# suoych/KEDs

Measured on AMD Instinct MI355X. Metric: query-images/sec (encode+0.5M top-10) ViT-L/14, higher is better.
Workload: dtype bf16/fp16 operands, fp32 accumulate; 1 GPU; ViT-L/14 encode_image (224x224 synthetic, random-init weights) + exact top-10 over a synthetic unit-norm 0.5M x 768 database; batch_per_gpu=128, global_batch=128, db_rows=500000, dim=768, k=10, parallelism=dp1 encoders + 1-way row-sharded scan

## Files before the change

### keds_amd/csrc/elementwise.hip

```cpp
#include "keds_common.h"
#include <math.h>

namespace {

constexpr float LN_EPS = 1e-5f;
constexpr int LN_MAXV = 8;

template <int OUT, int NV>
__global__ __launch_bounds__(256) void layernorm_kernel(const float* __restrict__ x, long long x_stride,
                                                        const int* __restrict__ row_map, int row_mul,
                                                        const float* __restrict__ gamma,
                                                        const float* __restrict__ beta, void* __restrict__ out,
                                                        int rows, int dim, long long pair_plane) {
    const int r = blockIdx.x * 4 + (threadIdx.x >> 6);
    const int lane = threadIdx.x & 63;
    if (r >= rows) return;
    const int rm = row_map ? row_map[r] : 0;
    const bool bad_row = row_map && (unsigned)rm >= (unsigned)row_mul;
    const long long src = (long long)r * row_mul + (bad_row ? 0 : rm);
    const float* p = x + src * x_stride;
    constexpr int MAXV = NV > 0 ? NV : LN_MAXV;
    f32x4 v[MAXV], gg[MAXV], bb[MAXV];
#pragma unroll
    for (int j = 0; j < MAXV; ++j) {
// ... 221 lines not shown
    float acc0 = 0.f, acc1 = 0.f, acc2 = 0.f;
    for (int y = ylo; y < yhi; ++y) {
        const float wy = pil_bicubic((y - yc + 0.5f) * yss) / wys;
        float h0 = 0.f, h1 = 0.f, h2 = 0.f;
        if (RW == W) {
            const unsigned char* p = src + ((size_t)y * W + (ox + left)) * 3;
            h0 = p[0]; h1 = p[1]; h2 = p[2];
        } else {
            const unsigned char* row = src + (size_t)y * W * 3;
            for (int x = xlo; x < xhi; ++x) {
                const float wx = pil_bicubic((x - xc + 0.5f) * xss) / wxs;
                h0 += wx * row[x * 3];
                h1 += wx * row[x * 3 + 1];
                h2 += wx * row[x * 3 + 2];
            }
            h0 = clip8(h0); h1 = clip8(h1); h2 = clip8(h2);
        }
        if (RH == H) {
            if (y == oy + top) { acc0 = h0; acc1 = h1; acc2 = h2; }
        } else {
            acc0 += wy * h0; acc1 += wy * h1; acc2 += wy * h2;
        }
    }
    if (RH != H) { acc0 = clip8(acc0); acc1 = clip8(acc1); acc2 = clip8(acc2); }
    const size_t plane = (size_t)n_px * n_px;
    float* o = out + (size_t)b * 3 * plane + (size_t)oy * n_px + ox;
    o[0] = (acc0 * (1.f / 255.f) - m0) / s0;
    o[plane] = (acc1 * (1.f / 255.f) - m1) / s1;
    o[2 * plane] = (acc2 * (1.f / 255.f) - m2) / s2;
}

__global__ __launch_bounds__(256) void preprocess_pil_kernel(const unsigned char* __restrict__ img, int B, int H, int W,
                                                             int n_px, int need_h, int need_v, int left, int top,
                                                             const int* __restrict__ xb, const int* __restrict__ xk, int ksx,
                                                             const int* __restrict__ yb, const int* __restrict__ yk, int ksy,
                                                             float m0, float m1, float m2, float s0, float s1, float s2,
                                                             float* __restrict__ out, unsigned char* __restrict__ out_u8) {
    const int idx = blockIdx.x * 256 + threadIdx.x;
    if (idx >= B * n_px * n_px) return;
    const int b = idx / (n_px * n_px), rem = idx - b * n_px * n_px;
    const int oy = rem / n_px, ox = rem - oy * n_px;
    const unsigned char* src = img + (size_t)b * H * W * 3;
    const int x0 = need_h ? xb[2 * ox] : ox + left, xn = need_h ? xb[2 * ox + 1] : 1;
    const int y0 = need_v ? yb[2 * oy] : oy + top, yn = need_v ? yb[2 * oy + 1] : 1;
    const int* kx = xk + (size_t)ox * ksx;
    const int* ky = yk + (size_t)oy * ksy;
    auto clip8 = [](int v) { v >>= 22; return v < 0 ? 0 : (v > 255 ? 255 : v); };
    int a0 = 1 << 21, a1 = 1 << 21, a2 = 1 << 21;
    int r0 = 0, r1 = 0, r2 = 0;
    for (int y = 0; y < yn; ++y) {
        const unsigned char* row = src + ((size_t)(y0 + y) * W + x0) * 3;
        int h0, h1, h2;
        if (need_h) {
            h0 = h1 = h2 = 1 << 21;
            for (int x = 0; x < xn; ++x) {
                const int k = kx[x];
                h0 += k * row[3 * x];
                h1 += k * row[3 * x + 1];
                h2 += k * row[3 * x + 2];
            }
            h0 = clip8(h0); h1 = clip8(h1); h2 = clip8(h2);
        } else {
            h0 = row[0]; h1 = row[1]; h2 = row[2];
        }
        if (need_v) {
            const int k = ky[y];
            a0 += k * h0; a1 += k * h1; a2 += k * h2;
        } else {
            r0 = h0; r1 = h1; r2 = h2;
        }
    }
    if (need_v) { r0 = clip8(a0); r1 = clip8(a1); r2 = clip8(a2); }
    const size_t plane = (size_t)n_px * n_px;
    float* o = out + (size_t)b * 3 * plane + (size_t)oy * n_px + ox;
    o[0] = ((float)r0 / 255.0f - m0) / s0;
    o[plane] = ((float)r1 / 255.0f - m1) / s1;
    o[2 * plane] = ((float)r2 / 255.0f - m2) / s2;
    if (out_u8) {
        unsigned char* u = out_u8 + ((size_t)b * plane + (size_t)oy * n_px + ox) * 3;
        u[0] = (unsigned char)r0; u[1] = (unsigned char)r1; u[2] = (unsigned char)r2;
    }
}

template <typename T>
__global__ __launch_bounds__(256) void im2col_kernel(const float* __restrict__ img, T* __restrict__ out, int R,
                                                     int P, int Kpad) {
    const int g = R / P;
    const int row = blockIdx.x;
    const int b = row / (g * g), pi = row % (g * g);
    const int py = pi / g, px = pi % g;
    const int kreal = 3 * P * P;
    const float* base = img + (size_t)b * 3 * R * R;
    for (int k = threadIdx.x; k < Kpad; k += 256) {
        float v = 0.f;
        if (k < kreal) {
            const int ch = k / (P * P), rem = k % (P * P);
            const int ky = rem / P, kx = rem % P;
            v = base[(size_t)ch * R * R + (size_t)(py * P + ky) * R + px * P + kx];
        }
        out[(size_t)row * Kpad + k] = (T)v;
    }
}

__global__ void cls_rows_kernel(float* __restrict__ x, const float* __restrict__ cls, const float* __restrict__ pos,
                                int B, int S, int d) {
    const int i = blockIdx.x * blockDim.x + threadIdx.x;
    if (i >= B * d) return;
    const int b = i / d, j = i % d;
    x[(size_t)b * S * d + j] = cls[j] + pos[j];
}

__global__ __launch_bounds__(256) void embed_tokens_kernel(const int* __restrict__ tokens,
                                                           const float* __restrict__ table,
                                                           const float* __restrict__ pos,
                                                           const float* __restrict__ img_tokens, int n_tok,
                                                           int insert_col, float* __restrict__ x, int L, int Lx, int d,
                                                           const int* __restrict__ seq_off) {
    const int b = blockIdx.x / Lx, t = blockIdx.x % Lx;
    size_t orow = (size_t)b * Lx + t;
    if (seq_off) {
        const int r0 = seq_off[b];
        if (t >= seq_off[b + 1] - r0) return;
        orow = (size_t)r0 + t;
    }
    const float* src;
    if (img_tokens && t >= insert_col && t < insert_col + n_tok) {
        src = img_tokens + ((size_t)b * n_tok + (t - insert_col)) * d;
    } else {
        const int col = (img_tokens && t >= insert_col + n_tok) ? t - (n_tok - 1) : t;
        src = table + (size_t)tokens[(size_t)b * L + col] * d;
    }
    const float* pe = pos + (size_t)t * d;
    float* o = x + orow * d;
    for (int i = threadIdx.x * 4; i < d; i += 1024)
        *reinterpret_cast<f32x4*>(o + i) =
            *reinterpret_cast<const f32x4*>(src + i) + *reinterpret_cast<const f32x4*>(pe + i);
}

__global__ __launch_bounds__(256) void l2norm_kernel(const float* __restrict__ x, float* __restrict__ out, int rows,
                                                     int dim) {
    const int r = blockIdx.x * 4 + (threadIdx.x >> 6);
    const int lane = threadIdx.x & 63;
    if (r >= rows) return;
    const float* p = x + (size_t)r * dim;
    float s = 0.f;
    for (int i = lane; i < dim; i += 64) s += p[i] * p[i];
    const float nrm = sqrtf(wave_sum(s));
    for (int i = lane; i < dim; i += 64) out[(size_t)r * dim + i] = p[i] / nrm;
}

__global__ __launch_bounds__(256) void mix_kernel(const float* __restrict__ a, const float* __restrict__ b, float wa,
                                                  float wb, float* __restrict__ an, float* __restrict__ bn,
                                                  float* __restrict__ mix, int rows, int dim) {
    const int r = blockIdx.x * 4 + (threadIdx.x >> 6);
    const int lane = threadIdx.x & 63;
    if (r >= rows) return;
    const float* pa = a + (size_t)r * dim;
    const float* pb = b + (size_t)r * dim;
    float sa = 0.f, sb = 0.f;
    for (int i = lane; i < dim; i += 64) {
        sa += pa[i] * pa[i];
        sb += pb[i] * pb[i];
    }
    const float na = sqrtf(wave_sum(sa)), nb = sqrtf(wave_sum(sb));
    float sm = 0.f;
    for (int i = lane; i < dim; i += 64) {
        const float m = wa * (pa[i] / na) + wb * (pb[i] / nb);
        sm += m * m;
    }
    const float nm = sqrtf(wave_sum(sm));
    for (int i = lane; i < dim; i += 64) {
        const float va = pa[i] / na, vb = pb[i] / nb;
        an[(size_t)r * dim + i] = va;
        bn[(size_t)r * dim + i] = vb;
        mix[(size_t)r * dim + i] = (wa * va + wb * vb) / nm;
    }
}

template <typename T>
__global__ void cast16_kernel(const float* __restrict__ x, T* __restrict__ out, long long n) {
    typedef __attribute__((ext_vector_type(4))) T t4;
    long long i = (blockIdx.x * (long long)blockDim.x + threadIdx.x) * 4;
    const long long step = (long long)gridDim.x * blockDim.x * 4;
// ... 170 lines not shown
    KedsProfScope prof(KEDS_PROF_OTHER, (hipStream_t)stream);
    const long long threads = (long long)rows * (cols / 8);
    split_f16_pair_kernel<<<(unsigned)((threads + 255) / 256), 256, 0, (hipStream_t)stream>>>(x, ld, rows, cols, (f16_t*)out, plane, overflow, 1.0f);
    return keds_check_launch("split_f16_pair_kernel");
}

extern "C" int keds_split_f16_weight(const float* w, int64_t n, int k, void* out, int64_t plane, int* w_exp, void* stream) {
    KEDS_REQUIRE(w && out && w_exp && n > 0 && k > 0 && k % 8 == 0 && plane >= n * k, "keds_split_f16_weight: bad argument");
    hipStream_t st = (hipStream_t)stream;
    unsigned* dmax = nullptr;
    if (hipMalloc(&dmax, sizeof(unsigned)) != hipSuccess) {
        keds_set_error("keds_split_f16_weight: out of device memory");
        return KEDS_E_LAUNCH;
    }
    unsigned hmax = 0;
    int rc = KEDS_OK;
    if (hipMemsetAsync(dmax, 0, sizeof(unsigned), st) != hipSuccess) rc = KEDS_E_LAUNCH;
    if (!rc) {
        absmax_bits_kernel<<<1024, 256, 0, st>>>(w, (long long)n * k, dmax);
        rc = keds_check_launch("absmax_bits_kernel");
    }
    if (!rc && (hipMemcpyAsync(&hmax, dmax, sizeof(unsigned), hipMemcpyDeviceToHost, st) != hipSuccess ||
                hipStreamSynchronize(st) != hipSuccess))
        rc = KEDS_E_LAUNCH;
    (void)hipFree(dmax);
    if (rc) {
        if (rc == KEDS_E_LAUNCH) keds_set_error("keds_split_f16_weight: device error while reading max |W|");
        return rc;
    }
    KEDS_REQUIRE(hmax < 0x7F800000u, "keds_split_f16_weight: the weight matrix holds a non-finite value");
    int e = 0;
    if (hmax) {
        const int lg = (int)(hmax >> 23) - 127;
        e = 13 - lg;
        if (e > 40) e = 40;
        if (e < -100) e = -100;
    }
    *w_exp = e;
    const long long threads = (long long)n * (k / 8);
    split_f16_pair_kernel<<<(unsigned)((threads + 255) / 256), 256, 0, st>>>(w, k, n, k, (f16_t*)out, plane, nullptr, ldexpf(1.0f, e));
    return keds_check_launch("split_f16_pair_kernel");
}

extern "C" int keds_layernorm(const float* x, int64_t x_stride, const float* gamma, const float* beta, void* out,
                              int out_f32, int rows, int dim, void* stream) {
    KEDS_REQUIRE(x && gamma && beta && out && rows > 0, "keds_layernorm: bad argument");
    KEDS_REQUIRE(ln_dim_ok(dim), "keds_layernorm: dim %d unsupported", dim);
    KEDS_REQUIRE(x_stride % 4 == 0, "keds_layernorm: row stride must be a multiple of 4");
    return keds_layernorm_impl(x, x_stride, nullptr, 1, gamma, beta, out, out_f32 ? 1 : 0, rows, dim, (hipStream_t)stream);
}

extern "C" int keds_layernorm_ex(const float* x, int64_t x_stride, const float* gamma, const float* beta, void* out,
                                 int out_type, int rows, int dim, void* stream) {
    KEDS_REQUIRE(out_type >= 0 && out_type <= 2, "keds_layernorm_ex: out_type %d (0 bf16, 1 fp32, 2 fp16)", out_type);
    KEDS_REQUIRE(x && gamma && beta && out && rows > 0, "keds_layernorm: bad argument");
    KEDS_REQUIRE(ln_dim_ok(dim), "keds_layernorm: dim %d unsupported", dim);
    KEDS_REQUIRE(x_stride % 4 == 0, "keds_layernorm: row stride must be a multiple of 4");
    return keds_layernorm_impl(x, x_stride, nullptr, 1, gamma, beta, out, out_type, rows, dim, (hipStream_t)stream);
}

extern "C" int keds_layernorm_rows(const float* x, int64_t x_stride, const int32_t* row_map, int row_mul, const float* gamma,
                                   const float* beta, void* out, int out_type, int rows, int dim, void* stream) {
    KEDS_REQUIRE(out_type >= 0 && out_type <= 2, "keds_layernorm_rows: out_type %d (0 bf16, 1 fp32, 2 fp16)", out_type);
    KEDS_REQUIRE(x && gamma && beta && out && rows > 0 && row_mul > 0, "keds_layernorm_rows: bad argument");
    KEDS_REQUIRE(ln_dim_ok(dim), "keds_layernorm_rows: dim %d unsupported", dim);
    KEDS_REQUIRE(x_stride % 4 == 0, "keds_layernorm_rows: row stride must be a multiple of 4");
    return keds_layernorm_impl(x, x_stride, row_map, row_mul, gamma, beta, out, out_type, rows, dim, (hipStream_t)stream);
}

extern "C" int keds_layernorm_pair(const float* x, int64_t x_stride, const float* gamma, const float* beta, void* out, int64_t plane,
                                   int rows, int dim, int form, void* stream) {
    KEDS_REQUIRE(x && gamma && beta && out && rows > 0 && (form == 0 || form == 1), "keds_layernorm_pair: bad argument");
    KEDS_REQUIRE(ln_dim_ok(dim), "keds_layernorm_pair: dim %d unsupported", dim);
    KEDS_REQUIRE(x_stride % 4 == 0, "keds_layernorm_pair: row stride must be a multiple of 4");
    KEDS_REQUIRE(plane % 4 == 0 && plane >= (int64_t)rows * dim, "keds_layernorm_pair: plane must be a multiple of 4 and hold rows * dim");
    return keds_layernorm_pair_impl(x, x_stride, gamma, beta, out, plane, rows, dim, (hipStream_t)stream, form);
}

extern "C" int keds_layernorm_pair_last_form(void) { return tl_ln_pair_form; }

extern "C" int keds_im2col_ex(const float* image, void* out, int out_f16, int B, int R, int P, int Kpad, void* stream) {
    KEDS_REQUIRE(image && out && B > 0 && P > 0 && R % P == 0, "keds_im2col: bad argument");
    KEDS_REQUIRE(Kpad >= 3 * P * P && Kpad % 64 == 0, "keds_im2col: Kpad must cover 3*P*P and be a multiple of 64");
    const int g = R / P;
    KedsProfScope prof(KEDS_PROF_OTHER, (hipStream_t)stream);
    if (out_f16) im2col_kernel<f16_t><<<B * g * g, 256, 0, (hipStream_t)stream>>>(image, (f16_t*)out, R, P, Kpad);
    else im2col_kernel<bf16_t><<<B * g * g, 256, 0, (hipStream_t)stream>>>(image, (bf16_t*)out, R, P, Kpad);
    return keds_check_launch("im2col_kernel");
}

extern "C" int keds_im2col(const float* image, void* out, int B, int R, int P, int Kpad, void* stream) {
    return keds_im2col_ex(image, out, 0, B, R, P, Kpad, stream);
}

int keds_cls_rows_impl(float* x, const float* cls, const float* pos, int B, int S, int d, hipStream_t st) {
    cls_rows_kernel<<<(B * d + 255) / 256, 256, 0, st>>>(x, cls, pos, B, S, d);
    return keds_check_launch("cls_rows_kernel");
}


extern "C" int keds_cls_rows(float* x, const float* cls, const float* pos, int B, int S, int d, void* stream) {
    KEDS_REQUIRE(x && cls && pos && B > 0 && S > 0 && d > 0, "keds_cls_rows: bad argument");
    return keds_cls_rows_impl(x, cls, pos, B, S, d, (hipStream_t)stream);
}

extern "C" int keds_embed_tokens_ex(const int32_t* tokens, const float* table, const float* pos, const float* img_tokens, int n_tok,
                                    int insert_col, float* x, int B, int L, int Lx, int d, const int32_t* seq_off, void* stream) {
    return keds_embed_tokens_impl(tokens, table, pos, img_tokens, n_tok, insert_col, x, B, L, Lx, d, stream, seq_off);
}

extern "C" int keds_embed_tokens(const int32_t* tokens, const float* table, const float* pos, const float* img_tokens,
                                 int n_tok, int insert_col, float* x, int B, int L, int d, void* stream) {
    return keds_embed_tokens_impl(tokens, table, pos, img_tokens, n_tok, insert_col, x, B, L, L, d, stream);
}

int keds_embed_tokens_impl(const int32_t* tokens, const float* table, const float* pos, const float* img_tokens,
                           int n_tok, int insert_col, float* x, int B, int L, int Lx, int d, void* stream, const int32_t* seq_off) {
    KEDS_REQUIRE(tokens && table && pos && x && B > 0 && L > 0 && Lx > 0 && Lx <= L, "keds_embed_tokens: bad argument");
    KEDS_REQUIRE(d % 4 == 0, "keds_embed_tokens: d must be a multiple of 4");
    if (img_tokens) {
        KEDS_REQUIRE(n_tok >= 1 && insert_col >= 0 && insert_col + n_tok <= L,
                     "keds_embed_tokens: splice [%d,%d) outside the context of %d", insert_col, insert_col + n_tok, L);
    }
    KedsProfScope prof(KEDS_PROF_OTHER, (hipStream_t)stream);
    embed_tokens_kernel<<<B * Lx, 256, 0, (hipStream_t)stream>>>(tokens, table, pos, img_tokens, n_tok, insert_col, x, L,
                                                                  Lx, d, seq_off);
    return keds_check_launch("embed_tokens_kernel");
}

extern "C" size_t keds_readout_workspace_bytes(int B, int d) {
    return keds_align_up((size_t)B, 128) * d * 2;
}

extern "C" int keds_readout(const float* x, int S, const int32_t* row, const float* gamma, const float* beta,
                            const void* proj_t, float* out, int B, int d, int E, int normalize, void* workspace,
                            size_t workspace_bytes, void* stream) {
    KEDS_REQUIRE(x && gamma && beta && proj_t && out && workspace && B > 0, "keds_readout: bad argument");
    KEDS_REQUIRE(ln_dim_ok(d), "keds_readout: d %d unsupported", d);
    if (workspace_bytes < keds_readout_workspace_bytes(B, d)) {
        keds_set_error("keds_readout: workspace too small");
        return KEDS_E_WORKSPACE;
    }
    return keds_run_readout(x, S, row, gamma, beta, proj_t, out, B, d, E, normalize, workspace, (hipStream_t)stream);
}

extern "C" int keds_l2_normalize(const float* x, float* out, int rows, int dim, void* stream) {
    KEDS_REQUIRE(x && out && rows > 0 && dim > 0, "keds_l2_normalize: bad argument");
    l2norm_kernel<<<(rows + 3) / 4, 256, 0, (hipStream_t)stream>>>(x, out, rows, dim);
    return keds_check_launch("l2norm_kernel");
}

extern "C" int keds_mix_normalize(const float* a, const float* b, float wa, float wb, float* a_n, float* b_n,
                                  float* mix, int rows, int dim, void* stream) {
    KEDS_REQUIRE(a && b && a_n && b_n && mix && rows > 0 && dim > 0, "keds_mix_normalize: bad argument");
    mix_kernel<<<(rows + 3) / 4, 256, 0, (hipStream_t)stream>>>(a, b, wa, wb, a_n, b_n, mix, rows, dim);
    return keds_check_launch("mix_kernel");
}

extern "C" int keds_cast_bf16(const float* x, void* out, int64_t count, void* stream) {
    KEDS_REQUIRE(x && out && count > 0, "keds_cast_bf16: bad argument");
    long long blocks = (count / 4 + 255) / 256;
    if (blocks > 4096) blocks = 4096;
    if (blocks < 1) blocks = 1;
    cast16_kernel<bf16_t><<<(unsigned)blocks, 256, 0, (hipStream_t)stream>>>(x, (bf16_t*)out, count);
    return keds_check_launch("cast16_kernel<bf16>");
}

extern "C" int keds_cast_f16(const float* x, void* out, int64_t count, void* stream) {
    KEDS_REQUIRE(x && out && count > 0, "keds_cast_f16: bad argument");
    long long blocks = (count / 4 + 255) / 256;
// ... 148 lines not shown
```

### keds_amd/csrc/gemm.hip

```cpp
#include "keds_common.h"
#include <math.h>
#include "gemm_shared.h"
#include "gemm_quad_gen.h"

#ifndef KEDS_QUAD_AUX_X
#define KEDS_QUAD_AUX_X 0
#endif
#ifndef KEDS_QUAD_AUX_W
#define KEDS_QUAD_AUX_W 0
#endif

namespace {

constexpr int BM = 128, BN = 128, BK = 64;
constexpr int TILE_BYTES = 128 * BK * 2;
constexpr int BUF_BYTES = 2 * TILE_BYTES;


__device__ __forceinline__ float qgelu(float x) {
    return x * __builtin_amdgcn_rcpf(1.0f + __builtin_amdgcn_exp2f(-2.4554669595930157f * x));
}

template <int EPI>
__device__ __forceinline__ void epilogue_store(f32x4 v0, f32x4 v1, void* __restrict__ out, int m, int n, int N,
// ... 268 lines not shown
            if constexpr (ND > 0) {
                if (16 * H + p * 8 + mi >= 32 - ND && defer) {
                    pend[16 * H + p * 8 + mi - (32 - ND)] = ov;
                    continue;
                }
            }
            keds_store16<KEDS_ST_LN>(ov, tile_out, off);
        }
    }
    if constexpr (epi_out_f16(EPI)) f16_range_flag(guard, rmax);
}
template <int ND>
__device__ __forceinline__ void quad_flush_pending(const u32x4* __restrict__ pend, char* __restrict__ tile_out, int N, int wm, int wn2,
                                                   int g, int c, int i0, int i1) {
    int r0 = 128 * wm + c;
    asm volatile("" : "+v"(r0));
#pragma unroll
    for (int i = 0; i < ND; ++i) {
        if (i < i0 || i >= i1) continue;
        const int s_ = 32 - ND + i, h = s_ >> 4, p = (s_ >> 3) & 1, mi = s_ & 7;
        const unsigned off = ((unsigned)(r0 + 16 * mi) * (unsigned)N + (unsigned)(64 * (2 * wn2 + h) + 32 * p + 8 * g)) * 2u;
        keds_store16<KEDS_ST_LN>(pend[i], tile_out, off);
    }
}

template <bool REDUCE = true>
__device__ __forceinline__ void pair_resid_epilogue(f32x4 (&acc)[4][8], const char* __restrict__ side, void* __restrict__ out,
                                                    int m0, int n0, int N, int wm, int wn, int g, int c,
                                                    keds_stat_t* __restrict__ stats, char* __restrict__ red) {
    const int r0 = 128 * wm + c;
    char* tile = reinterpret_cast<char*>(out) + ((size_t)m0 * N + n0) * 2;
    const int nl = 64 * wn + 8 * g;
    f16x8 r[2][8];
#if KEDS_LD_RESID_AUX
    const auto trs = __builtin_amdgcn_make_buffer_rsrc(tile, 0, 0x7FFFFFFF, 0x00020000);
#endif
#pragma unroll
    for (int p = 0; p < 2; ++p)
#pragma unroll
        for (int mi = 0; mi < 8; ++mi) {
#if KEDS_LD_RESID_AUX
            r[p][mi] = __builtin_bit_cast(f16x8, __builtin_amdgcn_raw_buffer_load_b128(
                           trs, (int)(((unsigned)(r0 + 16 * mi) * (unsigned)N + (unsigned)(nl + 32 * p)) * 2u), 0, KEDS_LD_RESID_AUX));
#else
            r[p][mi] = *reinterpret_cast<const f16x8*>(tile + ((unsigned)(r0 + 16 * mi) * (unsigned)N + (unsigned)(nl + 32 * p)) * 2u);
#endif
        }
    f32x4 b[2][2];
#pragma unroll
    for (int p = 0; p < 2; ++p) {
        b[p][0] = *reinterpret_cast<const f32x4*>(side + 2048 + (nl + 32 * p) * 4);
        b[p][1] = *reinterpret_cast<const f32x4*>(side + 2048 + (nl + 32 * p) * 4 + 16);
    }
    f32x2* rw = reinterpret_cast<f32x2*>(red) + wn * 256 + r0;
#pragma unroll
    for (int mi = 0; mi < 8; ++mi) {
        f32x4 sv = f32x4{0.f, 0.f, 0.f, 0.f}, qv = sv;
#pragma unroll
        for (int p = 0; p < 2; ++p) {
            const f16x8 q = r[p][mi];
            const f32x4 v0 = f32x4{(float)q[0], (float)q[1], (float)q[2], (float)q[3]} + (acc[2 * p][mi] + b[p][0]);
            const f32x4 v1 = f32x4{(float)q[4], (float)q[5], (float)q[6], (float)q[7]} + (acc[2 * p + 1][mi] + b[p][1]);
            const f16x8 ov = f16x8{(f16_t)v0[0], (f16_t)v0[1], (f16_t)v0[2], (f16_t)v0[3], (f16_t)v1[0], (f16_t)v1[1], (f16_t)v1[2], (f16_t)v1[3]};
            keds_store16<KEDS_ST_RESID>(ov, tile, ((unsigned)(r0 + 16 * mi) * (unsigned)N + (unsigned)(nl + 32 * p)) * 2u);
            sv = sv + (v0 + v1);
            qv = qv + (v0 * v0 + v1 * v1);
        }
        float s = (sv[0] + sv[1]) + (sv[2] + sv[3]), ss = (qv[0] + qv[1]) + (qv[2] + qv[3]);
        s = rows_sum(s);
        ss = rows_sum(ss);
        if (stats && g == 0) rw[16 * mi] = f32x2{s, ss};
    }
    if constexpr (REDUCE) {
        if (stats) {
            __syncthreads();
            const int t = threadIdx.x;
            if (t < 256) {
                const f32x2* rr = reinterpret_cast<const f32x2*>(red) + t;
                const f32x2 a = rr[0], b = rr[256], c2 = rr[512], d = rr[768];
                keds_stat_add(stats + 2 * (size_t)(m0 + t), (a[0] + b[0]) + (c2[0] + d[0]), (a[1] + b[1]) + (c2[1] + d[1]));
            }
        }
    }
}

__device__ __forceinline__ void pair_resid_epilogue_acc(f32x4 (&acc)[4][8], void* __restrict__ out, int m0, int n0, int N,
                                                        int wm, int wn, int g, int c, keds_stat_t* __restrict__ stats,
                                                        char* __restrict__ red) {
    const int r0 = 128 * wm + c;
    char* tile = reinterpret_cast<char*>(out) + ((size_t)m0 * N + n0) * 2;
    const int nl = 64 * wn + 8 * g;
    f32x2* rw = reinterpret_cast<f32x2*>(red) + wn * 256 + r0;
#pragma unroll
    for (int mi = 0; mi < 8; ++mi) {
        float s = 0.f, ss = 0.f;
#pragma unroll
        for (int p = 0; p < 2; ++p) {
            const f32x4 v0 = acc[2 * p][mi], v1 = acc[2 * p + 1][mi];
            const f16x8 ov = f16x8{(f16_t)v0[0], (f16_t)v0[1], (f16_t)v0[2], (f16_t)v0[3], (f16_t)v1[0], (f16_t)v1[1], (f16_t)v1[2], (f16_t)v1[3]};
            *reinterpret_cast<f16x8*>(tile + ((unsigned)(r0 + 16 * mi) * (unsigned)N + (unsigned)(nl + 32 * p)) * 2u) = ov;
            s += sum8(v0, v1);
            ss += sum8(v0 * v0, v1 * v1);
        }
        s = rows_sum(s);
        ss = rows_sum(ss);
        if (stats && g == 0) rw[16 * mi] = f32x2{s, ss};
    }
    if (stats) {
        __syncthreads();
        const int t = threadIdx.x;
        if (t < 256) {
            const f32x2* rr = reinterpret_cast<const f32x2*>(red) + t;
            const f32x2 a = rr[0], b = rr[256], c2 = rr[512], d = rr[768];
            keds_stat_add(stats + 2 * (size_t)(m0 + t), (a[0] + b[0]) + (c2[0] + d[0]), (a[1] + b[1]) + (c2[1] + d[1]));
        }
    }
}

template <int N>
__device__ __forceinline__ void small_wait_barrier() {
    asm volatile("s_waitcnt vmcnt(%0)\n\ts_barrier" ::"n"(N) : "memory");
}
template <int MAXAHEAD>
__device__ __forceinline__ void small_wait_stage(int ahead) {
    if constexpr (MAXAHEAD == 0) {
        small_wait_barrier<0>();
    } else {
        if (ahead >= MAXAHEAD) small_wait_barrier<MAXAHEAD * 8>();
        else small_wait_stage<MAXAHEAD - 1>(ahead);
    }
}

template <int EPI, int NST>
__global__ __launch_bounds__(256, 2) void gemm_bt_kernel(const bf16_t* __restrict__ X, const bf16_t* __restrict__ W,
                                                         const float* __restrict__ bias, void* __restrict__ out,
                                                         int M, int N, int K, int n_tiles,
                                                         const float* __restrict__ aux, int aux_i,
                                                         float* __restrict__ part, int k_len, int tiles, int m_pad,
                                                         long long lda, long long ldc, void* __restrict__ aux2,
                                                         int* __restrict__ guard, long long a_plane, long long w_plane) {
    extern __shared__ __attribute__((aligned(16))) char smem[];
    const int bid_all = xcd_remap(blockIdx.x, gridDim.x);
    const int ks = part ? bid_all / tiles : 0;
    const int bid = part ? bid_all - ks * tiles : bid_all;
    const int k_begin = ks * k_len;
    const int tm = bid / n_tiles, tn = bid - tm * n_tiles;
    const int m0 = tm * BM, n0 = tn * BN;
    const int tid = threadIdx.x, lane = tid & 63;
    const int wave = __builtin_amdgcn_readfirstlane(tid >> 6);
    const int wn = wave >> 1, wm = wave & 1;
    const int g = lane >> 4, c = lane & 15;

    const int srow = lane >> 3, sslot = lane & 7;
    auto xrs_ = __builtin_amdgcn_make_buffer_rsrc(const_cast<void*>(static_cast<const void*>(X + (size_t)m0 * lda)), 0, 0x7FFFFFFF, 0x00020000);
    auto wrs_ = __builtin_amdgcn_make_buffer_rsrc(const_cast<void*>(static_cast<const void*>(W + (size_t)n0 * K)), 0, 0x7FFFFFFF, 0x00020000);
    int xsrc[4], wsrc[4];
#pragma unroll
    for (int i = 0; i < 4; ++i) {
        const int R = 32 * wave + 8 * i + srow;
        const int ch = sslot ^ swz_f(R);
        const int xr = m0 + R < M ? R : M - 1 - m0;
        xsrc[i] = (int)((long long)xr * lda * 2) + ch * 16;
        wsrc[i] = perm_w(R) * K * 2 + ch * 16;
    }
    auto stage = [&](int buf, int kt) {
        char* xb = smem + buf * BUF_BYTES + (32 * wave) * 128;
// ... 318 lines not shown
            }
    }
    if constexpr (epi_is_ln(EPI)) {
        asm volatile("s_waitcnt vmcnt(16)" : "+v"(st_raw), "+v"(pb), "+v"(pc)::"memory");
        if (tid < 256) {
            float rs, nm;
            ln_coeff_from((keds_stat_t)(((unsigned long long)st_raw[1] << 32) | st_raw[0]),
                          (keds_stat_t)(((unsigned long long)st_raw[3] << 32) | st_raw[2]), 1.0f / (float)K, rs, nm,
                          n0 == 0 ? guard : nullptr);
            *reinterpret_cast<f32x2*>(smem + SIDE_OFF + tid * 8) = f32x2{rs, nm};
        } else {
            *reinterpret_cast<float*>(smem + SIDE_OFF + 2048 + (tid - 256) * 4) = pb;
            *reinterpret_cast<float*>(smem + SIDE_OFF + 3072 + (tid - 256) * 4) = pc;
        }
    }
    if constexpr (epi_resid16(EPI) && !RESID_IN) {
        if (tid >= 256) *reinterpret_cast<float*>(smem + SIDE_OFF + 2048 + (tid - 256) * 4) = pb;
    }
    if constexpr (RESID_IN) __builtin_amdgcn_sched_barrier(0);
    asm volatile("s_waitcnt vmcnt(8) lgkmcnt(0)\n\ts_barrier" ::: "memory");
    bf16x8 xf[8], wa[4], wb[4];
#pragma unroll
    for (int ni = 0; ni < 4; ++ni) wa[ni] = *reinterpret_cast<const bf16x8*>(smem + wrow + slot0 + ni * 2048);
#pragma unroll
    for (int mi = 0; mi < 8; ++mi) xf[mi] = *reinterpret_cast<const bf16x8*>(smem + xrow + slot0 + mi * 2048);

#define KEDS_PAIR_STEP(wc, wn_, nb, nslot, SYNC, ISSUE, ip, PREFETCH)                                          \
    {                                                                                                          \
        __builtin_amdgcn_sched_barrier(0);                                                                     \
        if constexpr (SYNC) asm volatile("s_waitcnt vmcnt(0) lgkmcnt(0)\n\ts_barrier" ::: "memory");           \
        __builtin_amdgcn_sched_barrier(0);                                                                     \
        _Pragma("unroll") for (int mi = 0; mi < 8; ++mi) {                                                     \
            _Pragma("unroll") for (int ni = 0; ni < 4; ++ni)                                                   \
                acc[ni][mi] = mma<epi_f16(EPI)>(wc[ni], xf[mi], acc[ni][mi]);                                  \
            if constexpr (PREFETCH) {                                                                          \
                if (mi == 0) {                                                                                 \
                    _Pragma("unroll") for (int ni = 0; ni < 4; ++ni)                                           \
                        wn_[ni] = *reinterpret_cast<const bf16x8*>((nb) + wrow + (nslot) + ni * 2048);         \
                }                                                                                              \
                xf[mi] = *reinterpret_cast<const bf16x8*>((nb) + xrow + (nslot) + mi * 2048);                  \
            }                                                                                                  \
            if constexpr (ISSUE) issue((ip), mi);                                                              \
        }                                                                                                      \
        if constexpr (PREFETCH) {                                                                              \
            __builtin_amdgcn_sched_group_barrier(0x008, 4, 0);                                                 \
            __builtin_amdgcn_sched_group_barrier(0x100, 5, 0);                                                 \
            if constexpr (ISSUE) __builtin_amdgcn_sched_group_barrier(0x020, 1, 0);                            \
            KEDS_PAIR_G(ISSUE) KEDS_PAIR_G(ISSUE) KEDS_PAIR_G(ISSUE) KEDS_PAIR_G(ISSUE) KEDS_PAIR_G(ISSUE)     \
            KEDS_PAIR_G(ISSUE) KEDS_PAIR_G(ISSUE)                                                              \
        }                                                                                                      \
    }
#define KEDS_PAIR_G(ISSUE)                                                                                     \
    __builtin_amdgcn_sched_group_barrier(0x008, 4, 0);                                                         \
    __builtin_amdgcn_sched_group_barrier(0x100, 1, 0);                                                         \
    if constexpr (ISSUE) __builtin_amdgcn_sched_group_barrier(0x020, 1, 0);

    int p = 0;
    for (; p + 2 < np; ++p) {
        const char* cb = smem + (p & 1) * PBUF_BYTES;
        const char* ob = smem + ((p + 1) & 1) * PBUF_BYTES;
        KEDS_PAIR_STEP(wa, wb, cb, slot1, false, false, 0, true)
        KEDS_PAIR_STEP(wb, wa, ob, slot0, true, true, p + 2, true)
    }
    {
        const char* cb = smem + (p & 1) * PBUF_BYTES;
        const char* ob = smem + ((p + 1) & 1) * PBUF_BYTES;
        KEDS_PAIR_STEP(wa, wb, cb, slot1, false, false, 0, true)
        KEDS_PAIR_STEP(wb, wa, ob, slot0, true, false, 0, true)
        KEDS_PAIR_STEP(wa, wb, ob, slot1, false, false, 0, true)
        KEDS_PAIR_STEP(wb, wa, ob, slot0, false, false, 0, false)
    }
#undef KEDS_PAIR_STEP
#undef KEDS_PAIR_G

    const bool zl = epi_is_ln(EPI) ? (n0 == 0 && wn == 0 && g == 0) : (g == 0);
    if constexpr (epi_is_ln(EPI))
        pair_ln_epilogue<EPI>(acc, smem + SIDE_OFF, out, m0, n0, N, wm, wn, g, c, aux2, nullptr, false, guard);
    else if constexpr (RESID_IN)
        pair_resid_epilogue_acc(acc, out, m0, n0, N, wm, wn, g, c, reinterpret_cast<keds_stat_t*>(const_cast<float*>(aux)),
                                smem + (np & 1) * PBUF_BYTES);
    else if constexpr (epi_resid16(EPI))
        pair_resid_epilogue(acc, smem + SIDE_OFF, out, m0, n0, N, wm, wn, g, c,
                            reinterpret_cast<keds_stat_t*>(const_cast<float*>(aux)), smem + (np & 1) * PBUF_BYTES);
    else
        tile_epilogue<EPI, 8>(acc, bias, out, m0 + 128 * wm + c, M, n0 + 64 * wn + 8 * g, N, K, aux, aux_i, aux2, N, zl, guard,
                              epi_x3(EPI) ? x3_wscale(w_plane) : 1.0f);
}

#ifndef KEDS_QUAD_ORDER
#define KEDS_QUAD_ORDER 1
#endif
#define KEDS_QMFMA(FIRST, j, mi, wc, xc)                                                                       \
    if constexpr (FIRST) {                                                                                     \
        if constexpr (epi_f16(EPI)) { KEDS_QUAD_MFMAZ_##j##_##mi("v_mfma_f32_16x16x32_f16", wc[j], xc[mi]) }   \
        else { KEDS_QUAD_MFMAZ_##j##_##mi("v_mfma_f32_16x16x32_bf16", wc[j], xc[mi]) }                         \
    } else {                                                                                                   \
        if constexpr (epi_f16(EPI)) { KEDS_QUAD_MFMA_##j##_##mi("v_mfma_f32_16x16x32_f16", wc[j], xc[mi]) }    \
        else { KEDS_QUAD_MFMA_##j##_##mi("v_mfma_f32_16x16x32_bf16", wc[j], xc[mi]) }                          \
    }
#if KEDS_QUAD_ORDER == 0
#define KEDS_QG2(FIRST, g_, a_, b_, wc, xc) KEDS_QMFMA(FIRST, a_, g_, wc, xc) KEDS_QMFMA(FIRST, b_, g_, wc, xc)
#else
#define KEDS_QG2(FIRST, g_, a_, b_, wc, xc) KEDS_QMFMA(FIRST, g_, a_, wc, xc) KEDS_QMFMA(FIRST, g_, b_, wc, xc)
#endif
#define KEDS_QRD(r_, xn, wn_, nb, nslot)                                                                       \
    if constexpr ((r_) < 8) xn[(r_) & 7] = *reinterpret_cast<const bf16x8*>((nb) + xrow + (nslot) + ((r_) & 7) * 2048); \
    else wn_[(r_) & 7] = *reinterpret_cast<const bf16x8*>((nb) + wrow + (nslot) + ((r_) & 7) * 2048);
#define KEDS_QGAP(n_, xn, wn_, nb, nslot, ISSUE, ip, PREFETCH)                                                 \
    if constexpr (ISSUE) {                                                                                     \
        if constexpr (((n_) & 1) == 0) {                                                                       \
            if constexpr ((int)(ISSUE) == 1 || (n_) < 16) issue((ip), (n_) >> 1);                              \
        } else if constexpr (PREFETCH) {                                                                       \
            KEDS_QRD((n_) >> 1, xn, wn_, nb, nslot)                                                            \
        }                                                                                                      \
    } else if constexpr (PREFETCH && (n_) < 16) {                                                              \
        KEDS_QRD(n_, xn, wn_, nb, nslot)                                                                       \
    }                                                                                                          \
    __builtin_amdgcn_sched_barrier(0);
#define KEDS_QUAD_GROUP(FIRST, mi, xc, wc, xn, wn_, nb, nslot, ISSUE, ip, PREFETCH)                            \
    KEDS_QG2(FIRST, mi, 0, 1, wc, xc) KEDS_QGAP(4 * (mi), xn, wn_, nb, nslot, ISSUE, ip, PREFETCH)             \
    KEDS_QG2(FIRST, mi, 2, 3, wc, xc) KEDS_QGAP(4 * (mi) + 1, xn, wn_, nb, nslot, ISSUE, ip, PREFETCH)         \
    KEDS_QG2(FIRST, mi, 4, 5, wc, xc) KEDS_QGAP(4 * (mi) + 2, xn, wn_, nb, nslot, ISSUE, ip, PREFETCH)         \
    KEDS_QG2(FIRST, mi, 6, 7, wc, xc) KEDS_QGAP(4 * (mi) + 3, xn, wn_, nb, nslot, ISSUE, ip, PREFETCH)
#define KEDS_QUAD_STEP(FIRST, xc, wc, xn, wn_, nb, nslot, SYNC, ISSUE, ip, PREFETCH)                           \
    {                                                                                                          \
        __builtin_amdgcn_sched_barrier(0);                                                                     \
        if constexpr ((int)(SYNC) >= 2)                                                                        \
            asm volatile("s_waitcnt vmcnt(%0) lgkmcnt(0)\n\ts_barrier" ::"n"((int)(SYNC) >= 2 ? (int)(SYNC) : 0) : "memory"); \
        else if constexpr (SYNC) asm volatile("s_waitcnt vmcnt(0) lgkmcnt(0)\n\ts_barrier" ::: "memory");       \
        __builtin_amdgcn_sched_barrier(0);                                                                     \
        KEDS_QUAD_GROUP(FIRST, 0, xc, wc, xn, wn_, nb, nslot, ISSUE, ip, PREFETCH)                             \
        KEDS_QUAD_GROUP(FIRST, 1, xc, wc, xn, wn_, nb, nslot, ISSUE, ip, PREFETCH)                             \
        KEDS_QUAD_GROUP(FIRST, 2, xc, wc, xn, wn_, nb, nslot, ISSUE, ip, PREFETCH)                             \
        KEDS_QUAD_GROUP(FIRST, 3, xc, wc, xn, wn_, nb, nslot, ISSUE, ip, PREFETCH)                             \
        KEDS_QUAD_GROUP(FIRST, 4, xc, wc, xn, wn_, nb, nslot, ISSUE, ip, PREFETCH)                             \
        KEDS_QUAD_GROUP(FIRST, 5, xc, wc, xn, wn_, nb, nslot, ISSUE, ip, PREFETCH)                             \
        KEDS_QUAD_GROUP(FIRST, 6, xc, wc, xn, wn_, nb, nslot, ISSUE, ip, PREFETCH)                             \
        KEDS_QUAD_GROUP(FIRST, 7, xc, wc, xn, wn_, nb, nslot, ISSUE, ip, PREFETCH)                             \
    }

namespace qd {
constexpr int SIDE0 = pr::SIDE_OFF;
constexpr int RED_OFF = pr::SIDE_OFF + 2 * 4096;
constexpr int LDS_BYTES = RED_OFF + 8192;
}

template <int EPI, int PERSIST = 0>
__global__ __launch_bounds__(256, 1) void gemm_bt_quad_kernel(const bf16_t* __restrict__ X, const bf16_t* __restrict__ W,
                                                              const float* __restrict__ bias, void* __restrict__ out,
                                                              int M, int N, int K, int n_tiles,
                                                              const float* __restrict__ aux, int aux_i,
                                                              void* __restrict__ aux2, int* __restrict__ guard, int ntiles,
                                                              long long a_plane = 0, long long w_plane = 0) {
    using namespace pr;
    extern __shared__ __attribute__((aligned(16))) char smem[];
    const int m_tiles = ntiles / n_tiles;
    const int tid = threadIdx.x, lane = tid & 63;
    const int wave = __builtin_amdgcn_readfirstlane(tid >> 6);
    const int wn2 = wave & 1, wm = wave >> 1;
    const int g = lane >> 4, c = lane & 15;

    const int R0 = 8 * wave + (lane >> 3);
    const int sch = (lane & 7) ^ swz_f(R0);
    const unsigned xoff = (unsigned)R0 * (unsigned)K * 2u + sch * 16;
    const unsigned woff = (unsigned)perm_w(R0) * (unsigned)K * 2u + sch * 16;
    const unsigned rstride = 32u * (unsigned)K * 2u;
// ... 620 lines not shown
```

### keds_amd/csrc/keds_common.h

```cpp
#pragma once
#include <hip/hip_runtime.h>
#include <hip/hip_ext.h>
#include <stdint.h>
#include <stddef.h>
#include <stdarg.h>
#include <stdio.h>
#include "../../include/keds_hip.h"

typedef __bf16 bf16_t;
typedef __attribute__((ext_vector_type(8))) __bf16 bf16x8;
typedef __attribute__((ext_vector_type(4))) __bf16 bf16x4;
typedef __attribute__((ext_vector_type(2))) __bf16 bf16x2;
typedef _Float16 f16_t;
typedef __attribute__((ext_vector_type(8))) _Float16 f16x8;
typedef __attribute__((ext_vector_type(4))) float f32x4;
typedef __attribute__((ext_vector_type(16))) float f32x16;
typedef __attribute__((ext_vector_type(4))) unsigned int u32x4;
typedef __attribute__((ext_vector_type(2))) unsigned int u32x2;

#define KEDS_WAVE 64

#include <cstdlib>

struct PackedRows {
// ... 54 lines not shown
bool keds_side_lane_enabled();
int keds_stream_order(hipStream_t from, hipEvent_t ev, hipStream_t to);
void keds_order_lock();
void keds_order_unlock();
int keds_stream_wait_locked(hipEvent_t ev, hipStream_t to);
struct AttnArgs {
    const void* qkv; void* out; int B, S, heads;
    void *q8, *s8; int q8_rows; const int32_t* seq_off;
    hipStream_t stream; hipEvent_t stop;
};
int keds_attention16(const AttnArgs& a, bool f16, int causal, int q_limit, bool* stop_taken = nullptr);

static inline size_t keds_align_up(size_t x, size_t a) { return (x + a - 1) / a * a; }
struct KedsCarver {
    char* base;
    size_t used = 0;
    char* take(size_t bytes) {
        char* p = base ? base + used : nullptr;
        used += keds_align_up(bytes, 256);
        return p;
    }
    size_t bytes() const { return used; }
};
static inline size_t rpad(size_t r) { return keds_align_up(r, 128); }

__attribute__((format(printf, 4, 5))) static inline int keds_launch_is_planned(const int (&want)[8], const int (&got)[8], const char* entry,
                                                                               const char* call_fmt, ...) {
    for (int i = 0; i < 8; ++i) {
        if (got[i] == want[i]) continue;
        char call[160];
        va_list ap;
        va_start(ap, call_fmt);
        vsnprintf(call, sizeof call, call_fmt, ap);
        va_end(ap);
        keds_set_error("%s: launched form differs from the plan at [%d]: %d, planned %d (%s)", entry, i, got[i], want[i], call);
        return KEDS_E_LAUNCH;
    }
    return KEDS_OK;
}

int keds_func_lds_once(const void* func, int bytes, const char* what);
int keds_device_cus();

#define KEDS_SPLITK_BYTES ((size_t)8 << 20)
struct KedsSplitKScope {
    float* prev_p;
    size_t prev_bytes;
    bool prev_off;
    KedsSplitKScope(void* p, size_t bytes);
    ~KedsSplitKScope();
};
void keds_splitk_scratch(float** p, size_t* bytes);

int keds_layernorm_impl(const float* x, long long x_stride, const int* row_map, int row_mul, const float* gamma,
                        const float* beta, void* out, int out_f32, int rows, int dim, hipStream_t st);
int keds_layernorm_pair_impl(const float* x, long long x_stride, const float* gamma, const float* beta, void* out, long long plane,
                             int rows, int dim, hipStream_t st, int form = 0);
int keds_cls_rows_impl(float* x, const float* cls, const float* pos, int B, int S, int d, hipStream_t st);
int keds_cast_rows_f16_f32_impl(const void* x16, float* x32, int rows, int dim, long long stride, hipStream_t st);
int keds_gather_rows_impl(const void* src, void* dst, const int32_t* row, int S, int B, int dim, int mode, hipStream_t st,
                          bool global_rows = false);
int keds_embed_tokens_impl(const int32_t* tokens, const float* table, const float* pos, const float* img_tokens,
                           int n_tok, int insert_col, float* x, int B, int L, int Lx, int d, void* stream,
                           const int32_t* seq_off = nullptr);
int keds_run_readout(const float* x, int S, const int32_t* row, const float* gamma, const float* beta, const void* proj_t, float* out,
                     int B, int d, int E, int normalize, void* workspace, hipStream_t st);
int attention_f32_impl(const float* qkv, float* out, int B, int S, int heads, int causal, int q_limit, const int32_t* seq_off,
                       void* stream);
int keds_attention_x3_impl(const float* qkv, float* out, void* pair, int64_t plane, int B, int S, int heads, int causal, int q_limit,
                           int* overflow, const int32_t* seq_off, void* stream);
int keds_l2norm_rows_f32_impl(float* x, int rows, int dim, hipStream_t st);
int keds_cross_core_f32_impl(const float* Q, const float* Kp, const float* Vp, float* out, int B, int K, int heads, hipStream_t st);

int* keds_numerics_guard();

bool keds_gemm_splits_rows(int M, int N, int K);

#ifndef KEDS_ST_LN
#define KEDS_ST_LN 3
#endif
#ifndef KEDS_ST_RESID
#define KEDS_ST_RESID 0
#endif
#ifndef KEDS_ST_ATTN
#define KEDS_ST_ATTN 0
#endif
#ifndef KEDS_ST_FP8_BF16
#define KEDS_ST_FP8_BF16 0
#endif
#ifndef KEDS_ST_FP8_MX
#define KEDS_ST_FP8_MX 0
#endif
#ifndef KEDS_ST_FP8_MXR
#define KEDS_ST_FP8_MXR 0
#endif
#ifndef KEDS_LD_ATTN_AUX
#define KEDS_LD_ATTN_AUX 0
#endif
#ifndef KEDS_LD_A3_AUX
#define KEDS_LD_A3_AUX 0
#endif
#ifndef KEDS_LD_RESID_AUX
#define KEDS_LD_RESID_AUX 0
#endif
template <int POLICY, typename T>
__device__ __forceinline__ void keds_store16(T v, void* base, unsigned off) {
    static_assert(sizeof(T) == 16, "16-byte stores only");
    if constexpr (POLICY == 0) {
        *reinterpret_cast<T*>(reinterpret_cast<char*>(base) + off) = v;
    } else if constexpr (POLICY >= 10 && POLICY < 20) {
        void* p = reinterpret_cast<char*>(base) + off;
        if constexpr (POLICY == 10) asm volatile("global_store_dwordx4 %0, %1, off\n\ts_nop 1" ::"v"(p), "v"(__builtin_bit_cast(u32x4, v)) : "memory");
        else if constexpr (POLICY == 11) asm volatile("global_store_dwordx4 %0, %1, off nt\n\ts_nop 1" ::"v"(p), "v"(__builtin_bit_cast(u32x4, v)) : "memory");
        else if constexpr (POLICY == 12) asm volatile("global_store_dwordx4 %0, %1, off sc0 sc1\n\ts_nop 1" ::"v"(p), "v"(__builtin_bit_cast(u32x4, v)) : "memory");
        else if constexpr (POLICY == 13) asm volatile("global_store_dwordx4 %0, %1, off sc1 nt\n\ts_nop 1" ::"v"(p), "v"(__builtin_bit_cast(u32x4, v)) : "memory");
        else asm volatile("global_store_dwordx4 %0, %1, off sc1\n\ts_nop 1" ::"v"(p), "v"(__builtin_bit_cast(u32x4, v)) : "memory");
    } else if constexpr (POLICY >= 20) {
        keds_store16<POLICY - 20>(v, base, off);
        __builtin_amdgcn_sched_barrier(0);
    } else {
        constexpr int aux = POLICY == 1 ? 2 : POLICY == 2 ? 17 : POLICY == 3 ? 18 : POLICY == 4 ? 16 : POLICY == 5 ? 19 : POLICY == 6 ? 1 : POLICY == 8 ? 0 : 3;
        const auto rs = __builtin_amdgcn_make_buffer_rsrc(base, 0, 0x7FFFFFFF, 0x00020000);
        __builtin_amdgcn_raw_buffer_store_b128(__builtin_bit_cast(u32x4, v), rs, (int)off, 0, aux);
    }
}

__device__ __forceinline__ float bf16_bits_to_f32(unsigned short b) {
    return __uint_as_float(((unsigned int)b) << 16);
}

__device__ __forceinline__ float wave_sum(float v) {
#pragma unroll
    for (int o = 32; o > 0; o >>= 1) v += __shfl_xor(v, o, 64);
    return v;
}
__device__ __forceinline__ float wave_max(float v) {
#pragma unroll
    for (int o = 32; o > 0; o >>= 1) v = fmaxf(v, __shfl_xor(v, o, 64));
    return v;
}

__device__ __forceinline__ float rows_max(float x) {
    auto a = __builtin_amdgcn_permlane16_swap(__float_as_uint(x), __float_as_uint(x), false, false);
    x = fmaxf(__uint_as_float(a[0]), __uint_as_float(a[1]));
    auto b = __builtin_amdgcn_permlane32_swap(__float_as_uint(x), __float_as_uint(x), false, false);
    return fmaxf(__uint_as_float(b[0]), __uint_as_float(b[1]));
}
__device__ __forceinline__ float rows_sum(float x) {
    auto a = __builtin_amdgcn_permlane16_swap(__float_as_uint(x), __float_as_uint(x), false, false);
    x = __uint_as_float(a[0]) + __uint_as_float(a[1]);
    auto b = __builtin_amdgcn_permlane32_swap(__float_as_uint(x), __float_as_uint(x), false, false);
    return __uint_as_float(b[0]) + __uint_as_float(b[1]);
}

__device__ __forceinline__ int xcd_remap(int bid, int nwg) {
    const int q = nwg >> 3, r = nwg & 7, x = bid & 7;
    const int base = (x < r) ? x * (q + 1) : r * (q + 1) + (x - r) * q;
    return base + (bid >> 3);
}

__device__ __forceinline__ void quad_tile_coords(int bid, int m_tiles, int n_tiles, int& tm, int& tn) {
    const int m8 = m_tiles & ~7;
    if (m8 && (n_tiles & 3) == 0 && bid < m8 * n_tiles) {
        const int grp = bid >> 5, within = bid & 31;
        const int grows = m8 >> 3;
        const int gn = grp / grows, gm = grp - gn * grows;
// ... 45 lines not shown
```

Baseline: 6825 query-images/sec.

## Stage im2col through LDS with vector loads and add patch-embed GEMM epilogue

The im2col kernel now processes one patch row (or a group of patches) per block. It loads image rows with vectorized float loads into an LDS tile converted to 16-bit, then writes output rows as 8-wide vector stores, where the old kernel did scalar strided gathers per element. A dedicated patch-embedding epilogue in the paired GEMM adds bias and positional embeddings and writes rows with the CLS offset, using scheduled load/store interleaving. These changes cut uncoalesced memory traffic in the patch-embed stage, which is a small share of the ViT-L encode, at the cost of LDS usage and new alignment requirements.

```diff
diff --git a/keds_amd/csrc/elementwise.hip b/keds_amd/csrc/elementwise.hip
--- a/keds_amd/csrc/elementwise.hip
+++ b/keds_amd/csrc/elementwise.hip
@@ -327,23 +327,44 @@
     }
 }
 
-template <typename T>
-__global__ __launch_bounds__(256) void im2col_kernel(const float* __restrict__ img, T* __restrict__ out, int R,
-                                                     int P, int Kpad) {
+template <typename T, int V>
+__global__ __launch_bounds__(256) void im2col_kernel(const float* __restrict__ img, T* __restrict__ out, int R, int P, int Kpad,
+                                                     int gp, int groups) {
+    extern __shared__ __attribute__((aligned(16))) unsigned char im2col_lds[];
+    T* tile = reinterpret_cast<T*>(im2col_lds);
+    typedef __attribute__((ext_vector_type(V))) float fvec;
+    typedef __attribute__((ext_vector_type(8))) T tvec8;
     const int g = R / P;
-    const int row = blockIdx.x;
-    const int b = row / (g * g), pi = row % (g * g);
-    const int py = pi / g, px = pi % g;
-    const int kreal = 3 * P * P;
-    const float* base = img + (size_t)b * 3 * R * R;
-    for (int k = threadIdx.x; k < Kpad; k += 256) {
-        float v = 0.f;
-        if (k < kreal) {
-            const int ch = k / (P * P), rem = k % (P * P);
-            const int ky = rem / P, kx = rem % P;
-            v = base[(size_t)ch * R * R + (size_t)(py * P + ky) * R + px * P + kx];
-        }
-        out[(size_t)row * Kpad + k] = (T)v;
+    const int grp = blockIdx.x % groups, bpy = blockIdx.x / groups;
+    const int b = bpy / g, py = bpy % g;
+    const int px0 = grp * gp, w = min(gp, g - px0);
+    const int W = gp * P, wv = w * P / V;
+    const float* src = img + ((size_t)b * 3 * R + (size_t)py * P) * R + (size_t)px0 * P;
+    const int nload = 3 * P * wv;
+#pragma unroll 4
+    for (int i = threadIdx.x; i < nload; i += 256) {
+        const int q = i / wv, xv = i - q * wv;
+        const int c = q / P, ky = q - c * P;
+        const fvec f = *reinterpret_cast<const fvec*>(src + ((size_t)c * R + ky) * R + xv * V);
+        T* t = tile + q * W + xv * V;
+#pragma unroll
+        for (int e = 0; e < V; ++e) t[e] = (T)f[e];
+    }
+    __syncthreads();
+    const int kreal = 3 * P * P, kv = Kpad / 8;
+    T* dst = out + ((size_t)bpy * g + px0) * Kpad;
+    const int nstore = w * kv;
+    for (int i = threadIdx.x; i < nstore; i += 256) {
+        const int p = i / kv, k0 = (i - p * kv) * 8;
+        int q = k0 / P, kx = k0 - q * P;
+        const T* t = tile + p * P;
+        tvec8 o;
+#pragma unroll
+        for (int e = 0; e < 8; ++e) {
+            o[e] = k0 + e < kreal ? t[q * W + kx] : (T)0.f;
+            if (++kx == P) kx = 0, ++q;
+        }
+        *reinterpret_cast<tvec8*>(dst + (size_t)i * 8) = o;
     }
 }
 
@@ -680,10 +701,32 @@
 extern "C" int keds_im2col_ex(const float* image, void* out, int out_f16, int B, int R, int P, int Kpad, void* stream) {
     KEDS_REQUIRE(image && out && B > 0 && P > 0 && R % P == 0, "keds_im2col: bad argument");
     KEDS_REQUIRE(Kpad >= 3 * P * P && Kpad % 64 == 0, "keds_im2col: Kpad must cover 3*P*P and be a multiple of 64");
+    KEDS_REQUIRE(((uintptr_t)out & 15) == 0, "keds_im2col: out must be 16-byte aligned");
+    KEDS_REQUIRE(6LL * P * P <= 65536, "keds_im2col: one patch (3*P*P 16-bit values) must fit 64 KB of LDS");
     const int g = R / P;
-    KedsProfScope prof(KEDS_PROF_OTHER, (hipStream_t)stream);
-    if (out_f16) im2col_kernel<f16_t><<<B * g * g, 256, 0, (hipStream_t)stream>>>(image, (f16_t*)out, R, P, Kpad);
-    else im2col_kernel<bf16_t><<<B * g * g, 256, 0, (hipStream_t)stream>>>(image, (bf16_t*)out, R, P, Kpad);
+    constexpr int TILE_ELEMS = 16384;
+    const int gpmax = std::min(g, std::max(1, TILE_ELEMS / (3 * P * P))), groups = (g + gpmax - 1) / gpmax;
+    const int gp = (g + groups - 1) / groups;
+    const size_t lds = (size_t)3 * P * gp * P * 2;
+    const bool split = groups > 1;
+    const int W = gp * P;
+    const int V = (R % 4 == 0 && (!split || W % 4 == 0) && ((uintptr_t)image & 15) == 0)  ? 4
+                  : (R % 2 == 0 && (!split || W % 2 == 0) && ((uintptr_t)image & 7) == 0) ? 2
+                                                                                           : 1;
+    const hipStream_t st = (hipStream_t)stream;
+    const int grid = B * g * groups;
+    KedsProfScope prof(KEDS_PROF_OTHER, st);
+#define KEDS_IM2COL(T, V) im2col_kernel<T, V><<<grid, 256, lds, st>>>(image, (T*)out, R, P, Kpad, gp, groups)
+    if (out_f16) {
+        if (V == 4) KEDS_IM2COL(f16_t, 4);
+        else if (V == 2) KEDS_IM2COL(f16_t, 2);
+        else KEDS_IM2COL(f16_t, 1);
+    } else {
+        if (V == 4) KEDS_IM2COL(bf16_t, 4);
+        else if (V == 2) KEDS_IM2COL(bf16_t, 2);
+        else KEDS_IM2COL(bf16_t, 1);
+    }
+#undef KEDS_IM2COL
     return keds_check_launch("im2col_kernel");
 }
 
diff --git a/keds_amd/csrc/gemm.hip b/keds_amd/csrc/gemm.hip
--- a/keds_amd/csrc/gemm.hip
+++ b/keds_amd/csrc/gemm.hip
@@ -374,6 +374,62 @@
             }
         }
     }
+}
+
+__device__ __forceinline__ void pair_patch_epilogue(f32x4 (&acc)[4][8], const float* __restrict__ bias, void* __restrict__ out,
+                                                    int m0, int n0, int N, int wm, int wn, int g, int c,
+                                                    const float* __restrict__ pos, int G) {
+    const int nl = 64 * wn + 8 * g;
+    const int t0 = m0 + m0 / G + 1;
+    char* tile = reinterpret_cast<char*>(out) + ((size_t)t0 * N + n0) * 4;
+    const char* ptile = reinterpret_cast<const char*>(pos + n0);
+    unsigned poff[8], ooff[8];
+#pragma unroll
+    for (int mi = 0; mi < 8; ++mi) {
+        const int m = m0 + 128 * wm + c + 16 * mi;
+        const int b = m / G, pidx = m - b * G;
+        poff[mi] = ((unsigned)(1 + pidx) * (unsigned)N + (unsigned)nl) * 4u;
+        ooff[mi] = ((unsigned)(m + b + 1 - t0) * (unsigned)N + (unsigned)nl) * 4u;
+    }
+    f32x4 bv[2][2];
+#pragma unroll
+    for (int p = 0; p < 2; ++p) {
+        bv[p][0] = bv[p][1] = f32x4{0.f, 0.f, 0.f, 0.f};
+        if (bias) {
+            bv[p][0] = *reinterpret_cast<const f32x4*>(bias + n0 + nl + 32 * p);
+            bv[p][1] = *reinterpret_cast<const f32x4*>(bias + n0 + nl + 32 * p + 4);
+        }
+    }
+    auto load = [&](int p, int h, f32x4 (&r)[4][2]) {
+#pragma unroll
+        for (int j = 0; j < 4; ++j) {
+            const char* s = ptile + poff[4 * h + j] + 128 * p;
+            r[j][0] = *reinterpret_cast<const f32x4*>(s);
+            r[j][1] = *reinterpret_cast<const f32x4*>(s + 16);
+        }
+    };
+    auto store = [&](int p, int h, f32x4 (&r)[4][2]) {
+#pragma unroll
+        for (int j = 0; j < 4; ++j) {
+            const int mi = 4 * h + j;
+            keds_store16<KEDS_ST_PATCH>((acc[2 * p][mi] + bv[p][0]) + r[j][0], tile, ooff[mi] + 128u * p);
+            keds_store16<KEDS_ST_PATCH>((acc[2 * p + 1][mi] + bv[p][1]) + r[j][1], tile, ooff[mi] + 128u * p + 16u);
+        }
+    };
+    f32x4 ra[4][2], rb[4][2];
+    load(0, 0, ra);
+    load(0, 1, rb);
+    __builtin_amdgcn_sched_barrier(0);
+    store(0, 0, ra);
+    __builtin_amdgcn_sched_barrier(0);
+    load(1, 0, ra);
+    __builtin_amdgcn_sched_barrier(0);
+    store(0, 1, rb);
+    __builtin_amdgcn_sched_barrier(0);
+    load(1, 1, rb);
+    __builtin_amdgcn_sched_barrier(0);
+    store(1, 0, ra);
+    store(1, 1, rb);
 }
 
 __device__ __forceinline__ void pair_resid_epilogue_acc(f32x4 (&acc)[4][8], void* __restrict__ out, int m0, int n0, int N,
@@ -858,6 +914,8 @@
     else if constexpr (epi_resid16(EPI))
         pair_resid_epilogue(acc, smem + SIDE_OFF, out, m0, n0, N, wm, wn, g, c,
                             reinterpret_cast<keds_stat_t*>(const_cast<float*>(aux)), smem + (np & 1) * PBUF_BYTES);
+    else if constexpr (epi_base(EPI) == KEDS_EPI_PATCH_F32)
+        pair_patch_epilogue(acc, bias, out, m0, n0, N, wm, wn, g, c, aux, aux_i);
     else
         tile_epilogue<EPI, 8>(acc, bias, out, m0 + 128 * wm + c, M, n0 + 64 * wn + 8 * g, N, K, aux, aux_i, aux2, N, zl, guard,
                               epi_x3(EPI) ? x3_wscale(w_plane) : 1.0f);
diff --git a/keds_amd/csrc/keds_common.h b/keds_amd/csrc/keds_common.h
--- a/keds_amd/csrc/keds_common.h
+++ b/keds_amd/csrc/keds_common.h
@@ -160,6 +160,9 @@
 #ifndef KEDS_ST_RESID
 #define KEDS_ST_RESID 0
 #endif
+#ifndef KEDS_ST_PATCH
+#define KEDS_ST_PATCH 0
+#endif
 #ifndef KEDS_ST_ATTN
 #define KEDS_ST_ATTN 0
 #endif
```

Measured after the change: 6825 query-images/sec, median of 2. No clear change (-0.0%).
